# r9y9/deepvoice3_pytorch

Hardware: NVIDIA H100
Metric: mel-frames/sec training step (B=16,T_mel=800) (higher is better)
Workload: dtype f32 via split 16-bit pairs (fp16 pairs forward, bf16 pairs for gradients; 3 wgmma passes per product, fp32 accumulate)

## Files before the change

### deepvoice3_pytorch_b200/csrc/tc_common.cuh

```cuda
#pragma once
#include <cuda.h>
#include <cuda_bf16.h>
#include "common.cuh"

namespace dv3 {
namespace tc {

__device__ __forceinline__ uint32_t smem_u32(const void* p) { return (uint32_t)__cvta_generic_to_shared(p); }

__device__ __forceinline__ void mbar_init(uint64_t* bar, uint32_t count) {
    asm volatile("mbarrier.init.shared::cta.b64 [%0], %1;" ::"r"(smem_u32(bar)), "r"(count));
}
__device__ __forceinline__ void fence_barrier_init() {
    asm volatile("fence.mbarrier_init.release.cluster;" ::: "memory");
}
__device__ __forceinline__ void fence_proxy_async() {
    asm volatile("fence.proxy.async.shared::cta;" ::: "memory");
}
__device__ __forceinline__ void mbar_arrive_expect_tx(uint64_t* bar, uint32_t bytes) {
    asm volatile("mbarrier.arrive.expect_tx.shared::cta.b64 _, [%0], %1;" ::"r"(smem_u32(bar)), "r"(bytes)
                 : "memory");
}
__device__ __forceinline__ void mbar_arrive(uint64_t* bar) {
    asm volatile("mbarrier.arrive.shared::cta.b64 _, [%0];" ::"r"(smem_u32(bar)) : "memory");
}
__device__ __forceinline__ void mbar_wait(uint64_t* bar, uint32_t parity) {
    asm volatile(
        "{\n"
        ".reg .pred p;\n"
        "DV3_WAIT:\n"
        "mbarrier.try_wait.parity.shared::cta.b64 p, [%0], %1;\n"
        "@p bra DV3_DONE;\n"
        "bra DV3_WAIT;\n"
        "DV3_DONE:\n"
        "}\n" ::"r"(smem_u32(bar)),
        "r"(parity)
        : "memory");
}

__device__ __forceinline__ void tma_load_3d(void* smem_dst, const CUtensorMap* map, uint64_t* bar, int c0, int c1,
                                            int c2) {
    asm volatile(
        "cp.async.bulk.tensor.3d.shared::cluster.global.mbarrier::complete_tx::bytes [%0], [%1, {%3, %4, %5}], [%2];"
        ::"r"(smem_u32(smem_dst)), "l"(map), "r"(smem_u32(bar)), "r"(c0), "r"(c1), "r"(c2)
        : "memory");
}
__device__ __forceinline__ void prefetch_tmap(const CUtensorMap* map) {
    asm volatile("prefetch.tensormap [%0];" ::"l"(map) : "memory");
}

template <int N>
__device__ __forceinline__ void setmaxnreg_dec() { asm volatile("setmaxnreg.dec.sync.aligned.u32 %0;" ::"n"(N)); }
template <int N>
__device__ __forceinline__ void setmaxnreg_inc() { asm volatile("setmaxnreg.inc.sync.aligned.u32 %0;" ::"n"(N)); }

__device__ __forceinline__ void wgmma_fence() { asm volatile("wgmma.fence.sync.aligned;" ::: "memory"); }
__device__ __forceinline__ void wgmma_commit() { asm volatile("wgmma.commit_group.sync.aligned;" ::: "memory"); }
template <int N>
__device__ __forceinline__ void wgmma_wait() { asm volatile("wgmma.wait_group.sync.aligned %0;" ::"n"(N) : "memory"); }
__device__ __forceinline__ int frag_row(int i, int warp_in_wg, int lane) {
    return 16 * warp_in_wg + (lane >> 2) + 8 * ((i >> 1) & 1);
}
__device__ __forceinline__ int frag_col(int i, int lane) { return 8 * (i >> 2) + 2 * (lane & 3) + (i & 1); }

__device__ __forceinline__ uint64_t make_wgmma_desc(uint32_t saddr, uint32_t lbo, uint32_t sbo, uint32_t layout) {
    uint64_t d = 0;
    d |= (uint64_t)((saddr & 0x3FFFF) >> 4);
    d |= (uint64_t)((lbo >> 4) & 0x3FFF) << 16;
    d |= (uint64_t)((sbo >> 4) & 0x3FFF) << 32;
    d |= (uint64_t)layout << 62;
    return d;
}
constexpr uint32_t WG_SW128 = 1, WG_SW64 = 2;

template <int TA, int TB>
__device__ __forceinline__ void wgmma_f16_n64(float* d, uint64_t a, uint64_t b, uint32_t acc) {
    asm volatile(
        "{\n.reg .pred p;\nsetp.ne.b32 p, %34, 0;\n"
        "wgmma.mma_async.sync.aligned.m64n64k16.f32.f16.f16 {%0, %1, %2, %3, %4, %5, %6, %7, %8, %9, %10, %11, %12, %13, %14, %15, %16, %17, %18, %19, %20, %21, %22, %23, %24, %25, %26, %27, %28, %29, %30, %31}, %32, %33, p, 1, 1, %35, %36;\n}\n"
        : "+f"(d[0]), "+f"(d[1]), "+f"(d[2]), "+f"(d[3]), "+f"(d[4]), "+f"(d[5]), "+f"(d[6]), "+f"(d[7]), "+f"(d[8]), "+f"(d[9]), "+f"(d[10]), "+f"(d[11]), "+f"(d[12]), "+f"(d[13]), "+f"(d[14]), "+f"(d[15]), "+f"(d[16]), "+f"(d[17]), "+f"(d[18]), "+f"(d[19]), "+f"(d[20]), "+f"(d[21]), "+f"(d[22]), "+f"(d[23]), "+f"(d[24]), "+f"(d[25]), "+f"(d[26]), "+f"(d[27]), "+f"(d[28]), "+f"(d[29]), "+f"(d[30]), "+f"(d[31])
        : "l"(a), "l"(b), "r"(acc), "n"(TA), "n"(TB));
// ... 56 lines not shown
```

### deepvoice3_pytorch_b200/csrc/tc_gemm.cu

```cuda
#include "tc_common.cuh"
#include "tc_ring.cuh"
#include "../../include/dv3b200.h"

namespace dv3 {

using namespace tc;

constexpr int TC_CONV_THREADS = 512;
constexpr int TC_PRODUCER_REGS = 24;
constexpr int TC_CONSUMER_REGS = 168;
constexpr int TC_EPILOGUE_REGS = 152;
static_assert(TC_PRODUCER_REGS <= 65536 / TC_CONV_THREADS && TC_CONSUMER_REGS >= 65536 / TC_CONV_THREADS &&
              TC_EPILOGUE_REGS >= 65536 / TC_CONV_THREADS, "setmaxnreg direction of each warpgroup");
static_assert(128 * TC_PRODUCER_REGS + 256 * TC_CONSUMER_REGS + 128 * TC_EPILOGUE_REGS <= 65536, "register file");
constexpr int MAX_TAPS_TC = 8;
enum { TC_GATED = 0, TC_CONV = 1 };

struct TcMaps { CUtensorMap a[2]; CUtensorMap b[2]; };

struct TcParams {
    int T;
    int Nc;
    int rows_per_tap;
    int k, kb_n;
    int tap_off[MAX_TAPS_TC];
    const float* bias; const float* spk; const float* res;
    float* y; float* save_a; float* save_s;
    int gate_mode, residual;
    float* out; const float* e1; const float* e2; float alpha; int addmode, relu;
    float p_drop; const unsigned long long* seed_ptr; uint32_t salt;
    float gmain;
    int operand_bf16;
};

template <int BK> struct SwizzleOf;
template <> struct SwizzleOf<64> { static constexpr uint32_t layout = WG_SW128, sbo = 1024; };
template <> struct SwizzleOf<32> { static constexpr uint32_t layout = WG_SW64, sbo = 512; };

template <int BK>
__device__ __forceinline__ uint64_t make_desc(uint32_t saddr) {
    return make_wgmma_desc(saddr, 16, SwizzleOf<BK>::sbo, SwizzleOf<BK>::layout);
}

template <int BR>
__device__ __forceinline__ void epilogue_gated(const TcParams& p, const float* arow, uint64_t* acc_empty, int a_row0,
                                               int a_z, int b_row0) {
    const int t = a_row0 + (threadIdx.x & 127), b = a_z, C = p.Nc;
    const bool tv = t < p.T;
    const float* __restrict__ bias = p.bias;
    const float* __restrict__ res = p.res;
    const float* __restrict__ spk = p.spk;
    float* __restrict__ yo = p.y;
    float* __restrict__ ao = p.save_a;
    float* __restrict__ so = p.save_s;
    const bool need_res = (p.gate_mode != 0) || p.residual;
    const size_t base = ((size_t)b * C + b_row0) * p.T + (tv ? t : 0);
#pragma unroll
    for (int c32 = 0; c32 < BR; c32 += 32) {
        float rr[32], sp[32];
        if (tv) {
            const size_t cb = base + (size_t)c32 * p.T;
#pragma unroll
            for (int i = 0; i < 32; ++i) rr[i] = need_res ? __ldg(&res[cb + (size_t)i * p.T]) : 0.f;
            if (spk) {
#pragma unroll
                for (int i = 0; i < 32; ++i) sp[i] = __ldg(&spk[cb + (size_t)i * p.T]);
            }
#pragma unroll
            for (int i = 0; i < 32; ++i) {
                const int c = b_row0 + c32 + i;
                const size_t idx = cb + (size_t)i * p.T;
                float va = arow[c32 + i];
                if (spk) va += sp[i];
                const float a = va + __ldg(&bias[c]);
                const float s = sigmoidf_(arow[BR + c32 + i] + __ldg(&bias[C + c]));
                float y;
                if (p.gate_mode == 0) {
                    y = a * s;
                    if (p.residual) y = (y + rr[i]) * 0.70710678118654752f;
                } else {
                    y = s * a + (1.f - s) * rr[i];
                }
                yo[idx] = y;
                if (ao) ao[idx] = a;
                if (so) so[idx] = s;
            }
        }
        if (c32 + 32 == BR) mbar_arrive(acc_empty);
    }
}

template <int NCOLS>
__device__ __forceinline__ void epilogue_conv(const TcParams& p, const float* arow, uint64_t* acc_empty, int a_row0,
                                              int a_z, int b_row0) {
    const int t = a_row0 + (threadIdx.x & 127), b = a_z;
    const bool tv = t < p.T;
    const DropCfg drop = make_drop(p.p_drop, p.seed_ptr, p.salt);
    const float* __restrict__ bias = p.bias;
    const float* __restrict__ e1 = p.e1;
    const float* __restrict__ e2 = p.e2;
    float* __restrict__ out = p.out;
#pragma unroll 1
    for (int c32 = 0; c32 < NCOLS; c32 += 32) {
        float d[32], v[32], x2[32];
#pragma unroll
        for (int i = 0; i < 32; ++i) d[i] = arow[c32 + i];
        if (c32 + 32 == NCOLS) mbar_arrive(acc_empty);
        const int n0 = b_row0 + c32;
        const size_t cb = ((size_t)b * p.Nc + n0) * p.T + (tv ? t : 0);
        if (tv) {
#pragma unroll
            for (int i = 0; i < 32; ++i) {
                const bool ok = n0 + i < p.Nc;
                v[i] = (p.addmode != 0 && ok) ? __ldg(&e1[cb + (size_t)i * p.T]) : 0.f;
                x2[i] = (p.addmode == 2 && ok) ? __ldg(&e2[cb + (size_t)i * p.T]) : 0.f;
            }
#pragma unroll
            for (int i = 0; i < 32; ++i) {
                const int n = n0 + i;
                if (n < p.Nc) {
                    const size_t idx = cb + (size_t)i * p.T;
                    float g = d[i] * drop_scale(drop, (uint32_t)idx);
                    if (bias) g += __ldg(&bias[n]);
                    if (p.addmode == 1) g += p.alpha * v[i];
                    else if (p.addmode == 2) g += v[i] * (1.f - x2[i]);
                    if (p.relu) g = fmaxf(g, 0.f);
                    out[idx] = g;
                }
            }
        }
    }
}

template <class Cfg, int NPL, class Decode, class Load, class Mma, class Gmain, class Epilogue>
__device__ __forceinline__ void tc_pipeline(const TcMaps& maps, int num_units, Decode decode, Load load, Mma mma,
                                            Gmain gmain, Epilogue epilogue) {
    static_assert(NPL == 1 || NPL == 2, "one or two operand planes");
    static_assert(Cfg::NCOLS <= 128, "main + cross accumulators must fit in the registers of a consumer thread");
    static_assert(Cfg::STAGES >= 2, "pipeline needs at least two stages");
    constexpr int STAGE = Cfg::STAGE, STAGES = Cfg::STAGES;
    constexpr int NR = Cfg::NCOLS / 2;
    pdl_trigger();
    extern __shared__ uint8_t smem_raw[];
    uint8_t* smem = reinterpret_cast<uint8_t*>((reinterpret_cast<uintptr_t>(smem_raw) + 1023) & ~(uintptr_t)1023);
    float* acc_tile = reinterpret_cast<float*>(smem + STAGES * STAGE);
    uint64_t* full = reinterpret_cast<uint64_t*>(smem + STAGES * STAGE + Cfg::ACC_TILE);
    uint64_t* empty = full + STAGES;
    uint64_t* acc_full = empty + STAGES;
    uint64_t* acc_empty = acc_full + 1;
    const int warp = threadIdx.x >> 5, lane = threadIdx.x & 31;

    if (threadIdx.x == 0) {
#pragma unroll
        for (int pl = 0; pl < NPL; ++pl) prefetch_tmap(&maps.a[pl]);
#pragma unroll
        for (int pl = 0; pl < NPL; ++pl) prefetch_tmap(&maps.b[pl]);
        for (int s = 0; s < STAGES; ++s) { mbar_init(&full[s], 1); mbar_init(&empty[s], 2); }
        mbar_init(acc_full, 256);
        mbar_init(acc_empty, 128);
        fence_barrier_init();
    }
    __syncthreads();
    pdl_wait();

    if (warp >= 12) {
        setmaxnreg_inc<TC_EPILOGUE_REGS>();
        int n = 0;
        for (int u = blockIdx.x; u < num_units; u += gridDim.x, ++n) {
            const auto w = decode(u);
            mbar_wait(acc_full, n & 1);
            epilogue(w, acc_tile, acc_empty);
        }
    } else if (warp >= 8) {
        setmaxnreg_dec<TC_PRODUCER_REGS>();
        if (warp == 8 && lane == 0) {
            int it = 0;
            for (int u = blockIdx.x; u < num_units; u += gridDim.x) {
                const auto w = decode(u);
                for (int kit = 0; kit < w.n_iters; ++kit, ++it) {
                    const int s = it % STAGES, ph = (it / STAGES) & 1;
                    mbar_wait(&empty[s], ph ^ 1);
                    mbar_arrive_expect_tx(&full[s], STAGE);
                    load(w, kit, smem + s * STAGE, &full[s]);
                }
            }
        }
    } else {
        setmaxnreg_inc<TC_CONSUMER_REGS>();
        const int wg = warp >> 2, wq = warp & 3;
        float acc[NR], xacc[NPL == 2 ? NR : 1];
        int it = 0, n = 0;
        for (int u = blockIdx.x; u < num_units; u += gridDim.x, ++n) {
            const auto w = decode(u);
#pragma unroll
            for (int i = 0; i < NR; ++i) {
                acc[i] = 0.f;
                if constexpr (NPL == 2) xacc[i] = 0.f;
            }
            for (int kit = 0; kit < w.n_iters; ++kit, ++it) {
                const int s = it % STAGES, ph = (it / STAGES) & 1;
                mbar_wait(&full[s], ph);
                wgmma_fence();
                mma(smem + s * STAGE, wg, acc, xacc);
                wgmma_commit();
                wgmma_wait<1>();
                if (kit > 0 && (threadIdx.x & 127) == 0) mbar_arrive(&empty[(it - 1) % STAGES]);
            }
            wgmma_wait<0>();
            if (w.n_iters > 0 && (threadIdx.x & 127) == 0) mbar_arrive(&empty[(it - 1) % STAGES]);
            const float gm = gmain(w);
            mbar_wait(acc_empty, (n & 1) ^ 1);
#pragma unroll
            for (int i = 0; i < NR; ++i) {
                float* dst = &acc_tile[(64 * wg + frag_row(i, wq, lane)) * Cfg::ACC_PITCH + frag_col(i, lane)];
                if constexpr (NPL == 2) *dst = fmaf(xacc[i], LO_INV, acc[i] * gm);
                else *dst = acc[i] * gm;
            }
            mbar_arrive(acc_full);
        }
    }
}

template <int MODE, int NBOX, int BR, int BK, bool BF16, int NPL>
__global__ void __launch_bounds__(TC_CONV_THREADS, 1)
tc_conv_kernel(const __grid_constant__ TcMaps maps, const __grid_constant__ TcParams p, int tiles_x, int tiles_y,
               int num_tiles) {
    using Cfg = TcCfg<NBOX, BK, BR, NPL>;
    constexpr int NCOLS = Cfg::NCOLS;
    constexpr int TILE = 128 * BK * 2, TILE_B = BR * BK * 2;
    constexpr int B_OFF = NPL * TILE;
    constexpr int A_HALF = 64 * BK * 2;
    const int n_iters = p.k * p.kb_n;

    struct Tile { int a_row0, a_z, b_row0, b_row1, n_iters; };
    auto decode = [&](int tile) {
        Tile w;
        const int ty = tile % tiles_y, r = tile / tiles_y;
        w.a_z = r / tiles_x;
        w.a_row0 = (r % tiles_x) * 128;
        if (MODE == TC_GATED) { w.b_row0 = ty * BR; w.b_row1 = p.Nc + ty * BR; }
        else { w.b_row0 = ty * BR * NBOX; w.b_row1 = w.b_row0 + BR; }
        w.n_iters = n_iters;
        return w;
    };
    auto load = [&](const Tile& w, int kit, uint8_t* st, uint64_t* bar) {
        const int j = kit / p.kb_n, kb = kit - j * p.kb_n;
        const int ax = kb * BK, ay = w.a_row0 + p.tap_off[j];
        const int by0 = j * p.rows_per_tap + w.b_row0, by1 = j * p.rows_per_tap + w.b_row1;
#pragma unroll
        for (int pl = 0; pl < NPL; ++pl) {
            tma_load_3d(st + pl * TILE, &maps.a[pl], bar, ax, ay, w.a_z);
            uint8_t* bdst = st + B_OFF + pl * NBOX * TILE_B;
            tma_load_3d(bdst, &maps.b[pl], bar, ax, by0, 0);
            if (NBOX == 2) tma_load_3d(bdst + TILE_B, &maps.b[pl], bar, ax, by1, 0);
        }
    };
    auto mma = [&](const uint8_t* st, int wg, float* acc, float* xacc) {
        const uint32_t sa = smem_u32(st) + wg * A_HALF, sb = smem_u32(st + B_OFF);
#pragma unroll
        for (int kk = 0; kk < BK / 16; ++kk) {
            const uint32_t ko = kk * 32;
            const uint64_t a0 = make_desc<BK>(sa + ko), b0 = make_desc<BK>(sb + ko);
            wgmma_mma<NCOLS, 0, 0>(BF16, acc, a0, b0, 1);
            if constexpr (NPL == 2) {
                const uint64_t a1 = make_desc<BK>(sa + TILE + ko), b1 = make_desc<BK>(sb + NBOX * TILE_B + ko);
                wgmma_mma<NCOLS, 0, 0>(BF16, xacc, a0, b1, 1);
                wgmma_mma<NCOLS, 0, 0>(BF16, xacc, a1, b0, 1);
            }
        }
    };
    auto gmain = [&](const Tile&) { return p.gmain; };
    auto epilogue = [&](const Tile& w, const float* acc_tile, uint64_t* acc_empty) {
        const float* arow = acc_tile + (threadIdx.x & 127) * Cfg::ACC_PITCH;
        if (MODE == TC_GATED) epilogue_gated<BR>(p, arow, acc_empty, w.a_row0, w.a_z, w.b_row0);
        else epilogue_conv<NCOLS>(p, arow, acc_empty, w.a_row0, w.a_z, w.b_row0);
    };
    tc_pipeline<Cfg, NPL>(maps, num_tiles, decode, load, mma, gmain, epilogue);
}

struct TcMnParams {
    int T, B, Mw, Nw, k;
    int tap_off[MAX_TAPS_TC];
    int nsplit, batches_per_split, kb_n;
    int tiles_n, tiles_m, num_units;
    float* dw; long long split_stride;
    int msplit; long long s_m, s_mh, s_n, s_j;
    float gcoef;
};

template <int NPL>
__global__ void __launch_bounds__(TC_CONV_THREADS, 1)
tc_wgrad_mn_kernel(const __grid_constant__ TcMaps maps, const __grid_constant__ TcMnParams p) {
    using Cfg = WgCfg<NPL>;
    constexpr int A_PL = 2 * WG_BOX, B_PL = 2 * WG_BOX;
    constexpr uint32_t LBO = 4096, SBO = 1024;

    struct Unit { int m0, n0, j, s, b_beg, n_iters; };
    auto decode = [&](int u) {
        Unit w;
        w.n0 = (u % p.tiles_n) * 128;
        int r = u / p.tiles_n;
        w.m0 = (r % p.tiles_m) * 128;
        r /= p.tiles_m;
        w.j = r % p.k;
        w.s = r / p.k;
        w.b_beg = w.s * p.batches_per_split;
        const int b_end = min(p.B, w.b_beg + p.batches_per_split);
        w.n_iters = (b_end > w.b_beg ? b_end - w.b_beg : 0) * p.kb_n;
        return w;
    };
    auto load = [&](const Unit& w, int kit, uint8_t* st, uint64_t* bar) {
        const int bi = kit / p.kb_n, tc_ = kit - bi * p.kb_n;
        const int b = w.b_beg + bi, t0 = tc_ * 32;
#pragma unroll
        for (int pl = 0; pl < NPL; ++pl) {
#pragma unroll
            for (int h = 0; h < 2; ++h)
                tma_load_3d(st + pl * A_PL + h * WG_BOX, &maps.a[pl], bar, w.m0 + h * 64, t0, b);
#pragma unroll
            for (int q = 0; q < 2; ++q)
                tma_load_3d(st + NPL * A_PL + pl * B_PL + q * WG_BOX, &maps.b[pl], bar, w.n0 + q * 64,
                            t0 + p.tap_off[w.j], b);
        }
    };
    auto mma = [&](const uint8_t* st, int wg, float* acc, float* xacc) {
        const uint32_t sa = smem_u32(st);
#pragma unroll
        for (int kk = 0; kk < 2; ++kk) {
            const uint32_t ko = kk * 16 * 128;
            const uint64_t a0 = make_wgmma_desc(sa + wg * WG_BOX + ko, LBO, SBO, WG_SW128);
            const uint64_t b0 = make_wgmma_desc(sa + NPL * A_PL + ko, LBO, SBO, WG_SW128);
            wgmma_mma<128, 1, 1>(true, acc, a0, b0, 1);
            if constexpr (NPL == 2) {
                const uint64_t a1 = make_wgmma_desc(sa + A_PL + wg * WG_BOX + ko, LBO, SBO, WG_SW128);
                const uint64_t b1 = make_wgmma_desc(sa + 2 * A_PL + B_PL + ko, LBO, SBO, WG_SW128);
                wgmma_mma<128, 1, 1>(true, xacc, a0, b1, 1);
                wgmma_mma<128, 1, 1>(true, xacc, a1, b0, 1);
            }
        }
    };
    auto gmain = [&](const Unit& w) { return 1.f + p.gcoef * (float)(2 * w.n_iters); };
    auto epilogue = [&](const Unit& w, const float* acc_tile, uint64_t* acc_empty) {
        const int r = threadIdx.x & 127;
        float* __restrict__ out = p.dw + (size_t)w.s * p.split_stride + (size_t)w.j * p.s_j;
        const int rows = min(128, p.Mw - w.m0), cols = min(128, p.Nw - w.n0);
        if (p.s_n == 1) {
            if (r < cols) {
                float* __restrict__ o = out + w.n0 + r;
#pragma unroll 4
                for (int i = 0; i < rows; ++i) {
                    const int m = w.m0 + i;
                    o[(size_t)(m % p.msplit) * p.s_m + (size_t)(m / p.msplit) * p.s_mh] = acc_tile[i * Cfg::ACC_PITCH + r];
                }
            }
        } else if (r < rows) {
            const int m = w.m0 + r;
            float* __restrict__ o = out + (size_t)(m % p.msplit) * p.s_m + (size_t)(m / p.msplit) * p.s_mh +
                                    (size_t)w.n0 * p.s_n;
            const float* arow = acc_tile + r * Cfg::ACC_PITCH;
#pragma unroll 4
            for (int c = 0; c < cols; ++c) o[(size_t)c * p.s_n] = arow[c];
        }
        mbar_arrive(acc_empty);
    };
    tc_pipeline<Cfg, NPL>(maps, p.num_units, decode, load, mma, gmain, epilogue);
}

typedef CUresult (*EncodeTiledFn)(CUtensorMap*, CUtensorMapDataType, cuuint32_t, void*, const cuuint64_t*,
                                  const cuuint64_t*, const cuuint32_t*, const cuuint32_t*, CUtensorMapInterleave,
                                  CUtensorMapSwizzle, CUtensorMapL2promotion, CUtensorMapFloatOOBfill);

static EncodeTiledFn encode_fn() {
    static const EncodeTiledFn fn = [] {
        void* f = nullptr;
        cudaDriverEntryPointQueryResult qres;
        cudaError_t e = cudaGetDriverEntryPoint("cuTensorMapEncodeTiled", &f, cudaEnableDefault, &qres);
        return (e == cudaSuccess) ? (EncodeTiledFn)f : (EncodeTiledFn) nullptr;
    }();
    return fn;
}

int encode_tmap_bf16_3d(CUtensorMap* map, const void* base, uint64_t d0, uint64_t d1, uint64_t d2,
                        uint64_t stride1_bytes, uint64_t stride2_bytes, uint32_t box0, uint32_t box1) {
    const EncodeTiledFn enc = encode_fn();
    if (!enc) { set_error("cuTensorMapEncodeTiled entry point unavailable"); return 1; }
    cuuint64_t dims[3] = {d0, d1, d2};
    cuuint64_t strides[2] = {stride1_bytes, stride2_bytes};
    cuuint32_t box[3] = {box0, box1, 1};
    cuuint32_t estr[3] = {1, 1, 1};
    const CUtensorMapSwizzle sw = box0 * 2 == 128 ? CU_TENSOR_MAP_SWIZZLE_128B : CU_TENSOR_MAP_SWIZZLE_64B;
    CUresult r = enc(map, CU_TENSOR_MAP_DATA_TYPE_BFLOAT16, 3, const_cast<void*>(base), dims, strides, box, estr,
                     CU_TENSOR_MAP_INTERLEAVE_NONE, sw, CU_TENSOR_MAP_L2_PROMOTION_L2_256B,
                     CU_TENSOR_MAP_FLOAT_OOB_FILL_NONE);
    if (r != CUDA_SUCCESS) {
        set_error("cuTensorMapEncodeTiled failed (%d): dims=(%llu,%llu,%llu) strides=(%llu,%llu) box=(%u,%u)", (int)r,
                  (unsigned long long)d0, (unsigned long long)d1, (unsigned long long)d2,
                  (unsigned long long)stride1_bytes, (unsigned long long)stride2_bytes, box0, box1);
        return 1;
    }
    return 0;
}

template <typename K>
static int ensure_smem(K kern, int bytes, const char* what) {
    cudaError_t e = cudaFuncSetAttribute(kern, cudaFuncAttributeMaxDynamicSharedMemorySize, bytes);
    if (e != cudaSuccess) { set_error("%s: cannot set %d B dynamic smem: %s", what, bytes, cudaGetErrorString(e)); return 1; }
    return 0;
}

template <class Cfg, auto kern, typename... Args>
static int launch_persistent(int units, cudaStream_t st, const char* what, const Args&... args) {
    static const int configured = ensure_smem(kern, Cfg::SMEM, what);
    if (configured) return 1;
    const int sms = config().sms, grid = units < sms ? units : sms;
    cudaError_t e = launch_k(kern, dim3(grid), dim3(TC_CONV_THREADS), (size_t)Cfg::SMEM, st, args...);
    if (e != cudaSuccess) { set_error("%s: launch failed: %s", what, cudaGetErrorString(e)); return 1; }
    return check_launch(what);
}

template <int MODE, int NBOX, int BR, int BK, bool BF16, int NPL>
static int launch_conv_fmt(const TcMaps& maps, const TcParams& p, int tiles_x, int tiles_y, int batch, cudaStream_t st,
                           const char* what) {
    const int num_tiles = tiles_x * tiles_y * batch;
    return launch_persistent<TcCfg<NBOX, BK, BR, NPL>, tc_conv_kernel<MODE, NBOX, BR, BK, BF16, NPL>>(
        num_tiles, st, what, maps, p, tiles_x, tiles_y, num_tiles);
}

template <int MODE, int NBOX, int BR, int BK, int NPL = 2>
static int launch_conv(const TcMaps& maps, const TcParams& p, int tiles_x, int tiles_y, int batch, cudaStream_t st,
                       const char* what) {
    if (p.operand_bf16)
        return launch_conv_fmt<MODE, NBOX, BR, BK, true, NPL>(maps, p, tiles_x, tiles_y, batch, st, what);
    return launch_conv_fmt<MODE, NBOX, BR, BK, false, NPL>(maps, p, tiles_x, tiles_y, batch, st, what);
}

static void fill_taps_tc(int* tap_off, int k, int dilation, int causal, bool transpose) {
    const int padl = causal ? (k - 1) * dilation : (k - 1) / 2 * dilation;
    for (int j = 0; j < MAX_TAPS_TC; ++j)
        tap_off[j] = j < k ? (transpose ? (padl - j * dilation) : (j * dilation - padl)) : 0;
}

static inline const void* plane(const void* base, int pl, long long plane_elems) {
    return (const char*)base + (size_t)pl * plane_elems * 2;
}

}

using namespace dv3;

extern "C" {

int dv3_tc_supported(int B, int C, int T, int k) {
    return (C % 128 == 0) && T >= 1 && k >= 1 && k <= MAX_TAPS_TC && B >= 1 && B <= 65535;
}
int dv3_tc_conv_supported(int B, int Cin, int Cout, int T, int k) {
    return T >= 1 && k >= 1 && k <= MAX_TAPS_TC && B >= 1 && B <= 65535 && (k == 1 || Cout % 128 == 0) && Cin >= 8 &&
           Cout >= 1;
}

int dv3_tc_convblock_fwd(const void* xd, const void* w, int npl, const float* bias, const float* spk,
                         const float* res, float* y, float* save_a, float* save_s, int B, int C, int T, int k,
                         int dilation, int causal, int mode, int residual, const void* fuse, void* stream) {
    DV3_REQUIRE(dv3_tc_supported(B, C, T, k), "tc_convblock_fwd: unsupported shape B=%d C=%d T=%d k=%d", B, C, T, k);
    DV3_REQUIRE(npl == 1 || npl == 2, "tc_convblock_fwd: npl must be 1 or 2");
    DV3_REQUIRE(fuse == nullptr, "tc_convblock_fwd: fuse must be NULL");
    TcMaps maps;
    const int t_tiles = (T + 127) / 128;
    const int BK = npl == 2 ? 32 : 64;
    for (int pl = 0; pl < npl; ++pl) {
        if (encode_tmap_bf16_3d(&maps.a[pl], plane(xd, pl, (long long)B * T * C), C, T, B, (uint64_t)C * 2,
                                (uint64_t)T * C * 2, BK, 128)) return 1;
        if (encode_tmap_bf16_3d(&maps.b[pl], plane(w, pl, (long long)k * 2 * C * C), C, (uint64_t)k * 2 * C, 1,
                                (uint64_t)C * 2, (uint64_t)k * 2 * C * C * 2, BK, 64)) return 1;
    }
    TcParams p = {};
    p.T = T; p.Nc = C; p.rows_per_tap = 2 * C; p.k = k; p.kb_n = C / BK;
    fill_taps_tc(p.tap_off, k, dilation, causal, false);
    p.bias = bias; p.spk = spk; p.res = res; p.y = y; p.save_a = save_a; p.save_s = save_s;
    p.gate_mode = mode; p.residual = residual;
    p.gmain = 1.f + config().tc_gamma * (float)(p.k * p.kb_n * (BK / 16));
    cudaStream_t st = (cudaStream_t)stream;
    if (npl == 1)
        return launch_conv_fmt<TC_GATED, 2, 64, 64, false, 1>(maps, p, t_tiles, C / 64, B, st, "tc_convblock_fwd");
    return launch_conv_fmt<TC_GATED, 2, 64, 32, false, 2>(maps, p, t_tiles, C / 64, B, st, "tc_convblock_fwd");
}

int dv3_tc_conv(const void* a, const void* w, int npl, float* out, int B, int Kc, int Nc, int T, int k, int dilation,
                int causal, int transpose_taps, const float* bias, int relu, float p_drop,
                const unsigned long long* seed_ptr, unsigned salt, int addmode, const float* e1, const float* e2,
                float alpha, const void* fuse, void* stream) {
    DV3_REQUIRE(k >= 1 && k <= MAX_TAPS_TC && (k == 1 || Nc % 128 == 0) && B <= 65535,
                "tc_conv: unsupported shape B=%d Kc=%d Nc=%d T=%d k=%d", B, Kc, Nc, T, k);
    DV3_REQUIRE(npl == 1 || npl == 2, "tc_conv: npl must be 1 or 2");
    DV3_REQUIRE(fuse == nullptr, "tc_conv: fuse must be NULL");
    const int Kp = (Kc + 7) / 8 * 8;
    const int t_tiles = (T + 127) / 128;
    cudaStream_t st = (cudaStream_t)stream;
    const long long tiles128 = (long long)t_tiles * ((Nc + 127) / 128) * B;
    const bool narrow = Nc > 64 && (k == 1 || Nc % 64 == 0) && tiles128 < 100;
    const bool k64 = Kc % 64 == 0;
    const int bk = ((narrow || npl == 1) && k64) ? 64 : 32, br = narrow ? 64 : 128;
    TcMaps maps;
    for (int pl = 0; pl < npl; ++pl) {
        if (encode_tmap_bf16_3d(&maps.a[pl], plane(a, pl, (long long)B * T * Kp), Kc, T, B, (uint64_t)Kp * 2,
                                (uint64_t)T * Kp * 2, bk, 128)) return 1;
        if (encode_tmap_bf16_3d(&maps.b[pl], plane(w, pl, (long long)k * Nc * Kp), Kc, (uint64_t)k * Nc, 1,
                                (uint64_t)Kp * 2, (uint64_t)k * Nc * Kp * 2, bk, br)) return 1;
    }
    TcParams p = {};
    p.T = T; p.Nc = Nc; p.rows_per_tap = Nc; p.k = k; p.kb_n = (Kc + bk - 1) / bk;
    fill_taps_tc(p.tap_off, k, dilation, causal, transpose_taps != 0);
    p.out = out; p.bias = bias; p.relu = relu; p.e1 = e1; p.e2 = e2; p.alpha = alpha; p.addmode = addmode;
    p.p_drop = p_drop; p.seed_ptr = seed_ptr; p.salt = salt;
    p.gmain = 1.f + config().tc_gamma * (float)(p.k * p.kb_n * (bk / 16));
    p.operand_bf16 = transpose_taps ? 1 : 0;
    const int tiles_y = (Nc + br - 1) / br;
    if (npl == 1) {
        if (narrow) {
            if (k64) return launch_conv<TC_CONV, 1, 64, 64, 1>(maps, p, t_tiles, tiles_y, B, st, "tc_conv(64)");
            return launch_conv<TC_CONV, 1, 64, 32, 1>(maps, p, t_tiles, tiles_y, B, st, "tc_conv(64,bk32)");
        }
        if (k64) return launch_conv<TC_CONV, 1, 128, 64, 1>(maps, p, t_tiles, tiles_y, B, st, "tc_conv(128,bk64)");
        return launch_conv<TC_CONV, 1, 128, 32, 1>(maps, p, t_tiles, tiles_y, B, st, "tc_conv(128)");
    }
    if (narrow) {
        if (k64) return launch_conv<TC_CONV, 1, 64, 64>(maps, p, t_tiles, tiles_y, B, st, "tc_conv(64)");
        return launch_conv<TC_CONV, 1, 64, 32>(maps, p, t_tiles, tiles_y, B, st, "tc_conv(64,bk32)");
    }
    return launch_conv<TC_CONV, 1, 128, 32>(maps, p, t_tiles, tiles_y, B, st, "tc_conv(128)");
}

constexpr double WG_UNIT_ITERS = 25.0;
constexpr double WG_SLAB_BYTES_PER_ITER = 1.5e6;
int dv3_tc_wgrad_nsplit(int B, int Mw, int Nw, int T, int k) {
    const long long tk = (long long)((Mw + 127) / 128) * ((Nw + 127) / 128) * k;
    const long long kb_n = (T + 31) / 32, sms = config().sms;
    const double slab = (double)Mw * Nw * k * 8.0 / WG_SLAB_BYTES_PER_ITER;
    auto cost = [&](int ns) {
        const long long bps = (B + ns - 1) / ns, U = tk * ns, U_full = tk * (ns - 1), G = U < sms ? U : sms;
        const long long L = bps * kb_n, L_last = (B - (ns - 1) * bps) * kb_n;
        return (double)((U_full + G - 1) / G) * (double)(L - L_last) +
               (double)((U + G - 1) / G) * ((double)L_last + WG_UNIT_ITERS) + ns * slab;
    };
    double best = 0.0;
    for (int bps = B, prev = 0; bps >= 1; --bps) {
        const int ns = (B + bps - 1) / bps;
        if (ns != prev && (prev == 0 || cost(ns) < best)) best = cost(ns);
        prev = ns;
    }
    for (int bps = B, prev = 0; bps >= 1; --bps) {
        const int ns = (B + bps - 1) / bps;
        if (ns != prev && cost(ns) <= 1.03 * best) return ns;
        prev = ns;
    }
    return 1;
}

int dv3_tc_wgrad_mn_npl(const void* dy, const void* xd, int npl, float* dw_partials, long long split_stride, int B,
                        int Mw, int Nw, int T, int k, int dilation, int causal, int msplit, long long s_m,
                        long long s_mh, long long s_n, long long s_j, void* stream) {
    DV3_REQUIRE(k >= 1 && k <= MAX_TAPS_TC && B <= 65535, "tc_wgrad_mn: unsupported shape k=%d", k);
    DV3_REQUIRE(npl == 1 || npl == 2, "tc_wgrad_mn: npl must be 1 or 2");
// ... 35 lines not shown
```

### deepvoice3_pytorch_b200/csrc/tc_ring.cuh

```cuda
#pragma once

namespace dv3 {

constexpr int SMEM_LIMIT = 232448;
constexpr int RING_SLACK = 1024 + 512;

template <int STAGE_BYTES, int TILE_COLS, int DEPTH>
struct RingCfg {
    static constexpr int STAGE = STAGE_BYTES;
    static constexpr int NCOLS = TILE_COLS;
    static constexpr int ACC_PITCH = NCOLS + 1;
    static constexpr int ACC_TILE = 128 * ACC_PITCH * 4;
    static constexpr int STAGES = DEPTH;
    static constexpr int SMEM = STAGES * STAGE + ACC_TILE + RING_SLACK;
    static constexpr int MAX_STAGES = (SMEM_LIMIT - ACC_TILE - RING_SLACK) / STAGE;
    static_assert(STAGE % 1024 == 0, "ring stages keep the 1 KB alignment of the swizzled TMA tiles");
    static_assert(STAGES >= 2, "pipeline needs at least two stages");
    static_assert(SMEM <= SMEM_LIMIT, "ring + hand-off tile + barriers exceed the 227 KB of a CTA");
};

template <int NBOX, int BK, int BR, int NPL> struct ConvRing;
template <> struct ConvRing<2, 32, 64, 2> { static constexpr int STAGES = 4; };
template <> struct ConvRing<1, 32, 128, 2> { static constexpr int STAGES = 4; };
template <> struct ConvRing<1, 64, 64, 2> { static constexpr int STAGES = 4; };
template <> struct ConvRing<1, 32, 64, 2> { static constexpr int STAGES = 6; };
template <> struct ConvRing<2, 64, 64, 1> { static constexpr int STAGES = 4; };
template <> struct ConvRing<1, 64, 128, 1> { static constexpr int STAGES = 4; };
template <> struct ConvRing<1, 32, 128, 1> { static constexpr int STAGES = 6; };
template <> struct ConvRing<1, 64, 64, 1> { static constexpr int STAGES = 6; };
template <> struct ConvRing<1, 32, 64, 1> { static constexpr int STAGES = 6; };

template <int NBOX, int BK, int BR, int NPL = 2>
using TcCfg = RingCfg<NPL * (128 + NBOX * BR) * BK * 2, BR * NBOX, ConvRing<NBOX, BK, BR, NPL>::STAGES>;

constexpr int WG_BOX = 64 * 32 * 2;
template <int NPL>
using WgCfg = RingCfg<NPL * 4 * WG_BOX, 128, NPL == 2 ? 5 : 6>;

}
```

Baseline: 1.597 million.

## Stage conv epilogue through swizzled smem tile and write outputs with TMA stores

The accumulator hand-off tile becomes a dense 128B-swizzled layout matching fp32 TMA boxes. The epilogue computes in place in shared memory and issues bulk tensor stores for y, save_a and save_s, replacing strided per-thread global stores along T. For gated blocks the residual is prefetched by TMA into a staging buffer for the next tile while the current one is processed. This adds shared-memory staging, extra barriers and a release that waits on bulk reads, which may delay freeing the accumulator tile.

```diff
diff --git a/deepvoice3_pytorch_b200/csrc/tc_common.cuh b/deepvoice3_pytorch_b200/csrc/tc_common.cuh
--- a/deepvoice3_pytorch_b200/csrc/tc_common.cuh
+++ b/deepvoice3_pytorch_b200/csrc/tc_common.cuh
@@ -47,6 +47,20 @@
 }
 __device__ __forceinline__ void prefetch_tmap(const CUtensorMap* map) {
     asm volatile("prefetch.tensormap [%0];" ::"l"(map) : "memory");
+}
+__device__ __forceinline__ void tma_store_3d(const CUtensorMap* map, const void* smem_src, int c0, int c1, int c2) {
+    asm volatile("cp.async.bulk.tensor.3d.global.shared::cta.bulk_group [%0, {%2, %3, %4}], [%1];"
+                 ::"l"(map), "r"(smem_u32(smem_src)), "r"(c0), "r"(c1), "r"(c2)
+                 : "memory");
+}
+__device__ __forceinline__ void bulk_commit() { asm volatile("cp.async.bulk.commit_group;" ::: "memory"); }
+__device__ __forceinline__ void bulk_wait_read() { asm volatile("cp.async.bulk.wait_group.read 0;" ::: "memory"); }
+__device__ __forceinline__ void bulk_wait() { asm volatile("cp.async.bulk.wait_group 0;" ::: "memory"); }
+__device__ __forceinline__ void mbar_arrive_cnt(uint64_t* bar, uint32_t count) {
+    asm volatile("mbarrier.arrive.shared::cta.b64 _, [%0], %1;" ::"r"(smem_u32(bar)), "r"(count) : "memory");
+}
+__device__ __forceinline__ void named_bar_sync(int id, int threads) {
+    asm volatile("bar.sync %0, %1;" ::"r"(id), "r"(threads) : "memory");
 }
 
 template <int N>
diff --git a/deepvoice3_pytorch_b200/csrc/tc_gemm.cu b/deepvoice3_pytorch_b200/csrc/tc_gemm.cu
--- a/deepvoice3_pytorch_b200/csrc/tc_gemm.cu
+++ b/deepvoice3_pytorch_b200/csrc/tc_gemm.cu
@@ -31,6 +31,7 @@
     float p_drop; const unsigned long long* seed_ptr; uint32_t salt;
     float gmain;
     int operand_bf16;
+    int tma_out;
 };
 
 template <int BK> struct SwizzleOf;
@@ -42,99 +43,170 @@
     return make_wgmma_desc(saddr, 16, SwizzleOf<BK>::sbo, SwizzleOf<BK>::layout);
 }
 
+
+template <int NC>
+__device__ __forceinline__ int dense_at(int c) {
+    const int r = threadIdx.x & 127;
+    return (r >> 5) * NC * 32 + c * 32 + ((((r >> 2) & 7) ^ (c & 7)) << 2) + (r & 3);
+}
+
+struct TcOutMaps { CUtensorMap out[3]; CUtensorMap res; };
+
+struct Handoff { float* tile; float* staging; uint64_t* acc_empty; uint64_t* in_full; };
+
+__device__ __forceinline__ void release_tile(const Handoff& h, bool tma) {
+    if (!tma) mbar_arrive(h.acc_empty);
+    else if ((threadIdx.x & 127) == 0) {
+        bulk_commit();
+        bulk_wait_read();
+        mbar_arrive_cnt(h.acc_empty, 128);
+    }
+}
+
 template <int BR>
-__device__ __forceinline__ void epilogue_gated(const TcParams& p, const float* arow, uint64_t* acc_empty, int a_row0,
+__device__ __forceinline__ void stage_residual(const TcParams& p, const TcOutMaps& om, const Handoff& h, int a_row0,
                                                int a_z, int b_row0) {
+    if (!p.tma_out || !((p.gate_mode != 0) || p.residual) || (threadIdx.x & 127) != 0) return;
+    mbar_arrive_expect_tx(h.in_full, 128 * BR * 4);
+#pragma unroll
+    for (int q = 0; q < 4; ++q) tma_load_3d(h.staging + q * BR * 32, &om.res, h.in_full, a_row0 + 32 * q, b_row0, a_z);
+}
+
+template <int BR>
+__device__ __forceinline__ void epilogue_gated(const TcParams& p, const TcOutMaps& om, const Handoff& h, int n,
+                                               int a_row0, int a_z, int b_row0) {
+    constexpr int NC = 2 * BR;
     const int t = a_row0 + (threadIdx.x & 127), b = a_z, C = p.Nc;
-    const bool tv = t < p.T;
+    const bool tv = t < p.T, tma = p.tma_out != 0;
     const float* __restrict__ bias = p.bias;
     const float* __restrict__ res = p.res;
     const float* __restrict__ spk = p.spk;
     float* __restrict__ yo = p.y;
     float* __restrict__ ao = p.save_a;
     float* __restrict__ so = p.save_s;
+    float* tile = h.tile;
+    float* st = h.staging;
     const bool need_res = (p.gate_mode != 0) || p.residual;
     const size_t base = ((size_t)b * C + b_row0) * p.T + (tv ? t : 0);
-#pragma unroll
+    if (need_res) {
+        if (tma) mbar_wait(h.in_full, n & 1);
+        else {
+#pragma unroll 8
+            for (int c = 0; c < BR; ++c) st[dense_at<BR>(c)] = tv ? __ldg(&res[base + (size_t)c * p.T]) : 0.f;
+        }
+    }
+#pragma unroll 1
     for (int c32 = 0; c32 < BR; c32 += 32) {
-        float rr[32], sp[32];
-        if (tv) {
-            const size_t cb = base + (size_t)c32 * p.T;
-#pragma unroll
-            for (int i = 0; i < 32; ++i) rr[i] = need_res ? __ldg(&res[cb + (size_t)i * p.T]) : 0.f;
-            if (spk) {
-#pragma unroll
-                for (int i = 0; i < 32; ++i) sp[i] = __ldg(&spk[cb + (size_t)i * p.T]);
-            }
-#pragma unroll
-            for (int i = 0; i < 32; ++i) {
-                const int c = b_row0 + c32 + i;
-                const size_t idx = cb + (size_t)i * p.T;
-                float va = arow[c32 + i];
-                if (spk) va += sp[i];
-                const float a = va + __ldg(&bias[c]);
-                const float s = sigmoidf_(arow[BR + c32 + i] + __ldg(&bias[C + c]));
-                float y;
-                if (p.gate_mode == 0) {
-                    y = a * s;
-                    if (p.residual) y = (y + rr[i]) * 0.70710678118654752f;
-                } else {
-                    y = s * a + (1.f - s) * rr[i];
-                }
-                yo[idx] = y;
-                if (ao) ao[idx] = a;
-                if (so) so[idx] = s;
-            }
-        }
-        if (c32 + 32 == BR) mbar_arrive(acc_empty);
-    }
+        float sp[32], ba[32], bb[32];
+        const size_t cb = base + (size_t)c32 * p.T;
+#pragma unroll
+        for (int i = 0; i < 32; ++i) {
+            ba[i] = __ldg(&bias[b_row0 + c32 + i]);
+            bb[i] = __ldg(&bias[C + b_row0 + c32 + i]);
+            if (spk) sp[i] = tv ? __ldg(&spk[cb + (size_t)i * p.T]) : 0.f;
+        }
+#pragma unroll
+        for (int i = 0; i < 32; ++i) {
+            const int cl = c32 + i;
+            float va = tile[dense_at<NC>(cl)];
+            if (spk) va += sp[i];
+            const float a = va + ba[i];
+            const float s = sigmoidf_(tile[dense_at<NC>(BR + cl)] + bb[i]);
+            const float rr = need_res ? st[dense_at<BR>(cl)] : 0.f;
+            float y;
+            if (p.gate_mode == 0) {
+                y = a * s;
+                if (p.residual) y = (y + rr) * 0.70710678118654752f;
+            } else {
+                y = s * a + (1.f - s) * rr;
+            }
+            st[dense_at<BR>(cl)] = y;
+            tile[dense_at<NC>(cl)] = a;
+            tile[dense_at<NC>(BR + cl)] = s;
+        }
+    }
+    if (tma) {
+        fence_proxy_async();
+        named_bar_sync(1, 128);
+        if ((threadIdx.x & 127) == 0) {
+#pragma unroll
+            for (int q = 0; q < 4; ++q) {
+                const int t0 = a_row0 + 32 * q;
+                if (t0 >= p.T) break;
+                tma_store_3d(&om.out[0], st + q * BR * 32, t0, b_row0, b);
+                if (ao) tma_store_3d(&om.out[1], tile + q * NC * 32, t0, b_row0, b);
+                if (so) tma_store_3d(&om.out[2], tile + q * NC * 32 + BR * 32, t0, b_row0, b);
+            }
+        }
+    } else if (tv) {
+#pragma unroll 8
+        for (int c = 0; c < BR; ++c) {
+            const size_t idx = base + (size_t)c * p.T;
+            yo[idx] = st[dense_at<BR>(c)];
+            if (ao) ao[idx] = tile[dense_at<NC>(c)];
+            if (so) so[idx] = tile[dense_at<NC>(BR + c)];
+        }
+    }
+    release_tile(h, tma);
 }
 
 template <int NCOLS>
-__device__ __forceinline__ void epilogue_conv(const TcParams& p, const float* arow, uint64_t* acc_empty, int a_row0,
+__device__ __forceinline__ void epilogue_conv(const TcParams& p, const TcOutMaps& om, const Handoff& h, int a_row0,
                                               int a_z, int b_row0) {
     const int t = a_row0 + (threadIdx.x & 127), b = a_z;
-    const bool tv = t < p.T;
+    const bool tv = t < p.T, tma = p.tma_out != 0;
     const DropCfg drop = make_drop(p.p_drop, p.seed_ptr, p.salt);
     const float* __restrict__ bias = p.bias;
     const float* __restrict__ e1 = p.e1;
     const float* __restrict__ e2 = p.e2;
     float* __restrict__ out = p.out;
+    float* tile = h.tile;
+    const size_t base = ((size_t)b * p.Nc + b_row0) * p.T + (tv ? t : 0);
 #pragma unroll 1
     for (int c32 = 0; c32 < NCOLS; c32 += 32) {
-        float d[32], v[32], x2[32];
-#pragma unroll
-        for (int i = 0; i < 32; ++i) d[i] = arow[c32 + i];
-        if (c32 + 32 == NCOLS) mbar_arrive(acc_empty);
+        float bz[32], v[32], x2[32];
         const int n0 = b_row0 + c32;
-        const size_t cb = ((size_t)b * p.Nc + n0) * p.T + (tv ? t : 0);
-        if (tv) {
-#pragma unroll
-            for (int i = 0; i < 32; ++i) {
-                const bool ok = n0 + i < p.Nc;
-                v[i] = (p.addmode != 0 && ok) ? __ldg(&e1[cb + (size_t)i * p.T]) : 0.f;
-                x2[i] = (p.addmode == 2 && ok) ? __ldg(&e2[cb + (size_t)i * p.T]) : 0.f;
-            }
-#pragma unroll
-            for (int i = 0; i < 32; ++i) {
-                const int n = n0 + i;
-                if (n < p.Nc) {
-                    const size_t idx = cb + (size_t)i * p.T;
-                    float g = d[i] * drop_scale(drop, (uint32_t)idx);
-                    if (bias) g += __ldg(&bias[n]);
-                    if (p.addmode == 1) g += p.alpha * v[i];
-                    else if (p.addmode == 2) g += v[i] * (1.f - x2[i]);
-                    if (p.relu) g = fmaxf(g, 0.f);
-                    out[idx] = g;
-                }
-            }
-        }
-    }
-}
-
-template <class Cfg, int NPL, class Decode, class Load, class Mma, class Gmain, class Epilogue>
+        const size_t cb = base + (size_t)c32 * p.T;
+#pragma unroll
+        for (int i = 0; i < 32; ++i) {
+            const bool ok = tv && n0 + i < p.Nc;
+            bz[i] = (bias && n0 + i < p.Nc) ? __ldg(&bias[n0 + i]) : 0.f;
+            v[i] = (p.addmode != 0 && ok) ? __ldg(&e1[cb + (size_t)i * p.T]) : 0.f;
+            x2[i] = (p.addmode == 2 && ok) ? __ldg(&e2[cb + (size_t)i * p.T]) : 0.f;
+        }
+#pragma unroll
+        for (int i = 0; i < 32; ++i) {
+            float& d = tile[dense_at<NCOLS>(c32 + i)];
+            float g = d * drop_scale(drop, (uint32_t)(cb + (size_t)i * p.T));
+            if (bias) g += bz[i];
+            if (p.addmode == 1) g += p.alpha * v[i];
+            else if (p.addmode == 2) g += v[i] * (1.f - x2[i]);
+            if (p.relu) g = fmaxf(g, 0.f);
+            d = g;
+        }
+    }
+    if (tma) {
+        fence_proxy_async();
+        named_bar_sync(1, 128);
+        if ((threadIdx.x & 127) == 0) {
+#pragma unroll
+            for (int q = 0; q < 4; ++q) {
+                const int t0 = a_row0 + 32 * q;
+                if (t0 >= p.T) break;
+                tma_store_3d(&om.out[0], tile + q * NCOLS * 32, t0, b_row0, b);
+            }
+        }
+    } else if (tv) {
+#pragma unroll 8
+        for (int c = 0; c < NCOLS; ++c)
+            if (b_row0 + c < p.Nc) out[base + (size_t)c * p.T] = tile[dense_at<NCOLS>(c)];
+    }
+    release_tile(h, tma);
+}
+
+template <class Cfg, int NPL, class Decode, class Load, class Mma, class Gmain, class Epilogue, class Stage>
 __device__ __forceinline__ void tc_pipeline(const TcMaps& maps, int num_units, Decode decode, Load load, Mma mma,
-                                            Gmain gmain, Epilogue epilogue) {
+                                            Gmain gmain, Epilogue epilogue, Stage stage) {
     static_assert(NPL == 1 || NPL == 2, "one or two operand planes");
     static_assert(Cfg::NCOLS <= 128, "main + cross accumulators must fit in the registers of a consumer thread");
     static_assert(Cfg::STAGES >= 2, "pipeline needs at least two stages");
@@ -142,12 +214,13 @@
     constexpr int NR = Cfg::NCOLS / 2;
     pdl_trigger();
     extern __shared__ uint8_t smem_raw[];
-    uint8_t* smem = reinterpret_cast<uint8_t*>((reinterpret_cast<uintptr_t>(smem_raw) + 1023) & ~(uintptr_t)1023);
+    uint8_t* smem = smem_raw + ((1024 - (smem_u32(smem_raw) & 1023)) & 1023);
     float* acc_tile = reinterpret_cast<float*>(smem + STAGES * STAGE);
-    uint64_t* full = reinterpret_cast<uint64_t*>(smem + STAGES * STAGE + Cfg::ACC_TILE);
+    uint64_t* full = reinterpret_cast<uint64_t*>(smem + STAGES * STAGE + Cfg::ACC_TILE + Cfg::STAGING);
     uint64_t* empty = full + STAGES;
     uint64_t* acc_full = empty + STAGES;
     uint64_t* acc_empty = acc_full + 1;
+    uint64_t* in_full = acc_empty + 1;
     const int warp = threadIdx.x >> 5, lane = threadIdx.x & 31;
 
     if (threadIdx.x == 0) {
@@ -158,6 +231,7 @@
         for (int s = 0; s < STAGES; ++s) { mbar_init(&full[s], 1); mbar_init(&empty[s], 2); }
         mbar_init(acc_full, 256);
         mbar_init(acc_empty, 128);
+        mbar_init(in_full, 1);
         fence_barrier_init();
     }
     __syncthreads();
@@ -165,12 +239,16 @@
 
     if (warp >= 12) {
         setmaxnreg_inc<TC_EPILOGUE_REGS>();
+        const Handoff h = {acc_tile, acc_tile + Cfg::ACC_TILE / 4, acc_empty, in_full};
+        if (blockIdx.x < num_units) stage(decode(blockIdx.x), h);
         int n = 0;
         for (int u = blockIdx.x; u < num_units; u += gridDim.x, ++n) {
             const auto w = decode(u);
             mbar_wait(acc_full, n & 1);
-            epilogue(w, acc_tile, acc_empty);
-        }
+            epilogue(w, n, h);
+            if (u + gridDim.x < num_units) stage(decode(u + gridDim.x), h);
+        }
+        if ((threadIdx.x & 127) == 0) bulk_wait();
     } else if (warp >= 8) {
         setmaxnreg_dec<TC_PRODUCER_REGS>();
         if (warp == 8 && lane == 0) {
@@ -210,9 +288,15 @@
             if (w.n_iters > 0 && (threadIdx.x & 127) == 0) mbar_arrive(&empty[(it - 1) % STAGES]);
             const float gm = gmain(w);
             mbar_wait(acc_empty, (n & 1) ^ 1);
+            const int sw = (((wq & 1) << 2) | (lane >> 4)) ^ ((lane & 3) << 1);
+            float* const frag0 = Cfg::DENSE ? acc_tile + (2 * wg + (wq >> 1)) * Cfg::NCOLS * 32 + (lane & 3) * 64 +
+                                                  ((lane >> 2) & 3)
+                                            : acc_tile;
 #pragma unroll
             for (int i = 0; i < NR; ++i) {
-                float* dst = &acc_tile[(64 * wg + frag_row(i, wq, lane)) * Cfg::ACC_PITCH + frag_col(i, lane)];
+                float* dst = Cfg::DENSE
+                    ? frag0 + (i >> 2) * 256 + (i & 1) * 32 + ((sw ^ (i & 3)) << 2)
+                    : &acc_tile[(64 * wg + frag_row(i, wq, lane)) * Cfg::ACC_PITCH + frag_col(i, lane)];
                 if constexpr (NPL == 2) *dst = fmaf(xacc[i], LO_INV, acc[i] * gm);
                 else *dst = acc[i] * gm;
             }
@@ -223,8 +307,8 @@
 
 template <int MODE, int NBOX, int BR, int BK, bool BF16, int NPL>
 __global__ void __launch_bounds__(TC_CONV_THREADS, 1)
-tc_conv_kernel(const __grid_constant__ TcMaps maps, const __grid_constant__ TcParams p, int tiles_x, int tiles_y,
-               int num_tiles) {
+tc_conv_kernel(const __grid_constant__ TcMaps maps, const __grid_constant__ TcOutMaps om,
+               const __grid_constant__ TcParams p, int tiles_x, int tiles_y, int num_tiles) {
     using Cfg = TcCfg<NBOX, BK, BR, NPL>;
     constexpr int NCOLS = Cfg::NCOLS;
     constexpr int TILE = 128 * BK * 2, TILE_B = BR * BK * 2;
@@ -270,12 +354,14 @@
         }
     };
     auto gmain = [&](const Tile&) { return p.gmain; };
-    auto epilogue = [&](const Tile& w, const float* acc_tile, uint64_t* acc_empty) {
-        const float* arow = acc_tile + (threadIdx.x & 127) * Cfg::ACC_PITCH;
-        if (MODE == TC_GATED) epilogue_gated<BR>(p, arow, acc_empty, w.a_row0, w.a_z, w.b_row0);
-        else epilogue_conv<NCOLS>(p, arow, acc_empty, w.a_row0, w.a_z, w.b_row0);
-    };
-    tc_pipeline<Cfg, NPL>(maps, num_tiles, decode, load, mma, gmain, epilogue);
+    auto epilogue = [&](const Tile& w, int n, const Handoff& h) {
+        if (MODE == TC_GATED) epilogue_gated<BR>(p, om, h, n, w.a_row0, w.a_z, w.b_row0);
+        else epilogue_conv<NCOLS>(p, om, h, w.a_row0, w.a_z, w.b_row0);
+    };
+    auto stage = [&](const Tile& w, const Handoff& h) {
+        if (MODE == TC_GATED) stage_residual<BR>(p, om, h, w.a_row0, w.a_z, w.b_row0);
+    };
+    tc_pipeline<Cfg, NPL>(maps, num_tiles, decode, load, mma, gmain, epilogue, stage);
 }
 
 struct TcMnParams {
@@ -340,7 +426,8 @@
         }
     };
     auto gmain = [&](const Unit& w) { return 1.f + p.gcoef * (float)(2 * w.n_iters); };
-    auto epilogue = [&](const Unit& w, const float* acc_tile, uint64_t* acc_empty) {
+    auto epilogue = [&](const Unit& w, int, const Handoff& h) {
+        const float* acc_tile = h.tile;
         const int r = threadIdx.x & 127;
         float* __restrict__ out = p.dw + (size_t)w.s * p.split_stride + (size_t)w.j * p.s_j;
         const int rows = min(128, p.Mw - w.m0), cols = min(128, p.Nw - w.n0);
@@ -361,9 +448,9 @@
 #pragma unroll 4
             for (int c = 0; c < cols; ++c) o[(size_t)c * p.s_n] = arow[c];
         }
-        mbar_arrive(acc_empty);
-    };
-    tc_pipeline<Cfg, NPL>(maps, p.num_units, decode, load, mma, gmain, epilogue);
+        mbar_arrive(h.acc_empty);
+    };
+    tc_pipeline<Cfg, NPL>(maps, p.num_units, decode, load, mma, gmain, epilogue, [](const Unit&, const Handoff&) {});
 }
 
 typedef CUresult (*EncodeTiledFn)(CUtensorMap*, CUtensorMapDataType, cuuint32_t, void*, const cuuint64_t*,
@@ -401,6 +488,25 @@
     return 0;
 }
 
+static int encode_tmap_f32_bct(CUtensorMap* map, const float* base, int B, int Nc, int T, int box_c) {
+    const EncodeTiledFn enc = encode_fn();
+    if (!enc) { set_error("cuTensorMapEncodeTiled entry point unavailable"); return 1; }
+    cuuint64_t dims[3] = {(cuuint64_t)T, (cuuint64_t)Nc, (cuuint64_t)B};
+    cuuint64_t strides[2] = {(cuuint64_t)T * 4, (cuuint64_t)Nc * T * 4};
+    cuuint32_t box[3] = {32, (cuuint32_t)box_c, 1};
+    cuuint32_t estr[3] = {1, 1, 1};
+    CUresult r = enc(map, CU_TENSOR_MAP_DATA_TYPE_FLOAT32, 3, const_cast<float*>(base), dims, strides, box, estr,
+                     CU_TENSOR_MAP_INTERLEAVE_NONE, CU_TENSOR_MAP_SWIZZLE_128B, CU_TENSOR_MAP_L2_PROMOTION_L2_256B,
+                     CU_TENSOR_MAP_FLOAT_OOB_FILL_NONE);
+    if (r != CUDA_SUCCESS) {
+        set_error("cuTensorMapEncodeTiled failed (%d): fp32 (B,C,T) = (%d,%d,%d) box=(32,%d)", (int)r, B, Nc, T, box_c);
+        return 1;
+    }
+    return 0;
+}
+
+static bool tma_rows(const float* base, int T) { return T % 4 == 0 && ((uintptr_t)base & 15) == 0; }
+
 template <typename K>
 static int ensure_smem(K kern, int bytes, const char* what) {
     cudaError_t e = cudaFuncSetAttribute(kern, cudaFuncAttributeMaxDynamicSharedMemorySize, bytes);
@@ -419,19 +525,19 @@
 }
 
 template <int MODE, int NBOX, int BR, int BK, bool BF16, int NPL>
-static int launch_conv_fmt(const TcMaps& maps, const TcParams& p, int tiles_x, int tiles_y, int batch, cudaStream_t st,
-                           const char* what) {
+static int launch_conv_fmt(const TcMaps& maps, const TcOutMaps& om, const TcParams& p, int tiles_x, int tiles_y,
+                           int batch, cudaStream_t st, const char* what) {
     const int num_tiles = tiles_x * tiles_y * batch;
     return launch_persistent<TcCfg<NBOX, BK, BR, NPL>, tc_conv_kernel<MODE, NBOX, BR, BK, BF16, NPL>>(
-        num_tiles, st, what, maps, p, tiles_x, tiles_y, num_tiles);
+        num_tiles, st, what, maps, om, p, tiles_x, tiles_y, num_tiles);
 }
 
 template <int MODE, int NBOX, int BR, int BK, int NPL = 2>
-static int launch_conv(const TcMaps& maps, const TcParams& p, int tiles_x, int tiles_y, int batch, cudaStream_t st,
-                       const char* what) {
+static int launch_conv(const TcMaps& maps, const TcOutMaps& om, const TcParams& p, int tiles_x, int tiles_y, int batch,
+                       cudaStream_t st, const char* what) {
     if (p.operand_bf16)
-        return launch_conv_fmt<MODE, NBOX, BR, BK, true, NPL>(maps, p, tiles_x, tiles_y, batch, st, what);
-    return launch_conv_fmt<MODE, NBOX, BR, BK, false, NPL>(maps, p, tiles_x, tiles_y, batch, st, what);
+        return launch_conv_fmt<MODE, NBOX, BR, BK, true, NPL>(maps, om, p, tiles_x, tiles_y, batch, st, what);
+    return launch_conv_fmt<MODE, NBOX, BR, BK, false, NPL>(maps, om, p, tiles_x, tiles_y, batch, st, what);
 }
 
 static void fill_taps_tc(int* tap_off, int k, int dilation, int causal, bool transpose) {
@@ -479,10 +585,20 @@
     p.bias = bias; p.spk = spk; p.res = res; p.y = y; p.save_a = save_a; p.save_s = save_s;
     p.gate_mode = mode; p.residual = residual;
     p.gmain = 1.f + config().tc_gamma * (float)(p.k * p.kb_n * (BK / 16));
+    const bool need_res = mode != 0 || residual;
+    TcOutMaps om = {};
+    p.tma_out = tma_rows(y, T) && (!save_a || tma_rows(save_a, T)) && (!save_s || tma_rows(save_s, T)) &&
+                (!need_res || tma_rows(res, T));
+    if (p.tma_out) {
+        const float* outs[3] = {y, save_a, save_s};
+        for (int i = 0; i < 3; ++i)
+            if (outs[i] && encode_tmap_f32_bct(&om.out[i], outs[i], B, C, T, 64)) return 1;
+        if (need_res && encode_tmap_f32_bct(&om.res, res, B, C, T, 64)) return 1;
+    }
     cudaStream_t st = (cudaStream_t)stream;
     if (npl == 1)
-        return launch_conv_fmt<TC_GATED, 2, 64, 64, false, 1>(maps, p, t_tiles, C / 64, B, st, "tc_convblock_fwd");
-    return launch_conv_fmt<TC_GATED, 2, 64, 32, false, 2>(maps, p, t_tiles, C / 64, B, st, "tc_convblock_fwd");
+        return launch_conv_fmt<TC_GATED, 2, 64, 64, false, 1>(maps, om, p, t_tiles, C / 64, B, st, "tc_convblock_fwd");
+    return launch_conv_fmt<TC_GATED, 2, 64, 32, false, 2>(maps, om, p, t_tiles, C / 64, B, st, "tc_convblock_fwd");
 }
 
 int dv3_tc_conv(const void* a, const void* w, int npl, float* out, int B, int Kc, int Nc, int T, int k, int dilation,
@@ -514,20 +630,23 @@
     p.p_drop = p_drop; p.seed_ptr = seed_ptr; p.salt = salt;
     p.gmain = 1.f + config().tc_gamma * (float)(p.k * p.kb_n * (bk / 16));
     p.operand_bf16 = transpose_taps ? 1 : 0;
+    TcOutMaps om = {};
+    p.tma_out = tma_rows(out, T);
+    if (p.tma_out && encode_tmap_f32_bct(&om.out[0], out, B, Nc, T, br)) return 1;
     const int tiles_y = (Nc + br - 1) / br;
     if (npl == 1) {
         if (narrow) {
-            if (k64) return launch_conv<TC_CONV, 1, 64, 64, 1>(maps, p, t_tiles, tiles_y, B, st, "tc_conv(64)");
-            return launch_conv<TC_CONV, 1, 64, 32, 1>(maps, p, t_tiles, tiles_y, B, st, "tc_conv(64,bk32)");
-        }
-        if (k64) return launch_conv<TC_CONV, 1, 128, 64, 1>(maps, p, t_tiles, tiles_y, B, st, "tc_conv(128,bk64)");
-        return launch_conv<TC_CONV, 1, 128, 32, 1>(maps, p, t_tiles, tiles_y, B, st, "tc_conv(128)");
+            if (k64) return launch_conv<TC_CONV, 1, 64, 64, 1>(maps, om, p, t_tiles, tiles_y, B, st, "tc_conv(64)");
+            return launch_conv<TC_CONV, 1, 64, 32, 1>(maps, om, p, t_tiles, tiles_y, B, st, "tc_conv(64,bk32)");
+        }
+        if (k64) return launch_conv<TC_CONV, 1, 128, 64, 1>(maps, om, p, t_tiles, tiles_y, B, st, "tc_conv(128,bk64)");
+        return launch_conv<TC_CONV, 1, 128, 32, 1>(maps, om, p, t_tiles, tiles_y, B, st, "tc_conv(128)");
     }
     if (narrow) {
-        if (k64) return launch_conv<TC_CONV, 1, 64, 64>(maps, p, t_tiles, tiles_y, B, st, "tc_conv(64)");
-        return launch_conv<TC_CONV, 1, 64, 32>(maps, p, t_tiles, tiles_y, B, st, "tc_conv(64,bk32)");
-    }
-    return launch_conv<TC_CONV, 1, 128, 32>(maps, p, t_tiles, tiles_y, B, st, "tc_conv(128)");
+        if (k64) return launch_conv<TC_CONV, 1, 64, 64>(maps, om, p, t_tiles, tiles_y, B, st, "tc_conv(64)");
+        return launch_conv<TC_CONV, 1, 64, 32>(maps, om, p, t_tiles, tiles_y, B, st, "tc_conv(64,bk32)");
+    }
+    return launch_conv<TC_CONV, 1, 128, 32>(maps, om, p, t_tiles, tiles_y, B, st, "tc_conv(128)");
 }
 
 constexpr double WG_UNIT_ITERS = 25.0;
diff --git a/deepvoice3_pytorch_b200/csrc/tc_ring.cuh b/deepvoice3_pytorch_b200/csrc/tc_ring.cuh
--- a/deepvoice3_pytorch_b200/csrc/tc_ring.cuh
+++ b/deepvoice3_pytorch_b200/csrc/tc_ring.cuh
@@ -5,18 +5,21 @@
 constexpr int SMEM_LIMIT = 232448;
 constexpr int RING_SLACK = 1024 + 512;
 
-template <int STAGE_BYTES, int TILE_COLS, int DEPTH>
+template <int STAGE_BYTES, int TILE_COLS, int DEPTH, bool DENSE_TILE = false, int STAGING_BYTES = 0>
 struct RingCfg {
     static constexpr int STAGE = STAGE_BYTES;
     static constexpr int NCOLS = TILE_COLS;
-    static constexpr int ACC_PITCH = NCOLS + 1;
+    static constexpr bool DENSE = DENSE_TILE;
+    static constexpr int ACC_PITCH = DENSE ? NCOLS : NCOLS + 1;
     static constexpr int ACC_TILE = 128 * ACC_PITCH * 4;
+    static constexpr int STAGING = STAGING_BYTES;
     static constexpr int STAGES = DEPTH;
-    static constexpr int SMEM = STAGES * STAGE + ACC_TILE + RING_SLACK;
-    static constexpr int MAX_STAGES = (SMEM_LIMIT - ACC_TILE - RING_SLACK) / STAGE;
+    static constexpr int SMEM = STAGES * STAGE + ACC_TILE + STAGING + RING_SLACK;
+    static constexpr int MAX_STAGES = (SMEM_LIMIT - ACC_TILE - STAGING - RING_SLACK) / STAGE;
     static_assert(STAGE % 1024 == 0, "ring stages keep the 1 KB alignment of the swizzled TMA tiles");
+    static_assert(ACC_TILE % 1024 == 0 || !DENSE, "the dense tile and the staging buffer are swizzled TMA boxes");
     static_assert(STAGES >= 2, "pipeline needs at least two stages");
-    static_assert(SMEM <= SMEM_LIMIT, "ring + hand-off tile + barriers exceed the 227 KB of a CTA");
+    static_assert(SMEM <= SMEM_LIMIT, "ring + hand-off tile + staging + barriers exceed the 227 KB of a CTA");
 };
 
 template <int NBOX, int BK, int BR, int NPL> struct ConvRing;
@@ -31,7 +34,8 @@
 template <> struct ConvRing<1, 32, 64, 1> { static constexpr int STAGES = 6; };
 
 template <int NBOX, int BK, int BR, int NPL = 2>
-using TcCfg = RingCfg<NPL * (128 + NBOX * BR) * BK * 2, BR * NBOX, ConvRing<NBOX, BK, BR, NPL>::STAGES>;
+using TcCfg = RingCfg<NPL * (128 + NBOX * BR) * BK * 2, BR * NBOX, ConvRing<NBOX, BK, BR, NPL>::STAGES, true,
+                      NBOX == 2 ? 128 * BR * 4 : 0>;
 
 constexpr int WG_BOX = 64 * 32 * 2;
 template <int NPL>
```

Result: faster. 1.687 million, median of 6 (+5.7%).
